# nanograv/PTMCMCSampler

Measured on AMD Instinct MI355X. Metric: MH updates/sec (whole node) + ESS/sec, 100-d Gaussian, 64 temps x 4096 walkers per GPU, higher is better.
Workload: dtype f64

## Files before the change

ptmcmcsampler_amd/csrc/ptmi_mh.inc.h:

```cpp
#pragma once
#include <stdlib.h>

#include "ptmi_common.h"

template <bool STR, int J>
__device__ __forceinline__ u64 grp_bcast(u64 v)
{
    if (STR) return (u64)__shfl((long long)v, (int)(threadIdx.x & 15) + 16 * J, 64);
    return quad_bcast<J>(v);
}
template <bool STR, int J>
__device__ __forceinline__ double grp_bcastf(double v)
{
    if (STR) return __shfl(v, (int)(threadIdx.x & 15) + 16 * J, 64);
    return quad_bcastf<J>(v);
}
template <int G, bool STR>
__device__ __forceinline__ double grp_sum(double p)
{
    if (STR) {
        p = p + __shfl_xor(p, 32, 64);
        p = p + __shfl_xor(p, 16, 64);
        return p;
    }
// ... 1092 lines not shown
    double cd_c = 0.0, cd_n = 0.0;

    constexpr bool PIPE = PAIRED && PERS != 0 && !FULL && !GRP && LOGL == PTMI_LOGL_ISO && PRI == PTMI_LOGP_FLAT;
    double x[EPL], dq[EPL], urow[PIPE ? EPL : 1];
#pragma unroll
    for (int e = 0; e < EPL; ++e) PTMI_ROW_LOAD(x[e], xrow, e);
    double lnL = a.lnL[ch], lp = a.lp[ch];
    u32 nacc = 0, jp[PTMI_J_FUSED] = {0, 0, 0}, ja[PTMI_J_FUSED] = {0, 0, 0};
    long long am_next = (FULL && a.am_base != nullptr) ? a.am_base[ch] : 0;
    const bool cold = live && tg == 0 && a.AM != nullptr;
    int am_row = a.am_row0;
    double box_margin = -1.0;
    double box_guard = 0.0;

    constexpr bool SQUAD = SCAMFAST && ScamBatch<STR, GW>::QUAD;
    constexpr bool PASSES = GW > 4 || SQUAD;
    constexpr int KPASS = GW > 4 ? GW / 2 : (SQUAD ? 4 : (1 << 30));
    constexpr int STM = (PERS || TLDS) ? 1 : (ULDS ? 2 : 0);
    auto scam_root_s = [&](int kk) {
        if (ULDS && !ulds_box) return smem[d * d + kk];
        return det_sqrt(S[kk]);
    };
    [[maybe_unused]] int koff = 0;
    [[maybe_unused]] auto row_request = [&](int off) __attribute__((always_inline)) {
        if constexpr (PIPE) {
            const double *row = smem + off;
            const ptmi_d2 *rp = reinterpret_cast<const ptmi_d2 *>(row) + gl;
#pragma unroll
            for (int e2 = 0; e2 < EPL / 2; ++e2) { const ptmi_d2 v = rp[4 * e2]; urow[2 * e2] = v.x; urow[2 * e2 + 1] = v.y; }
            if (EPL & 1) urow[EPL - 1] = row[8 * (EPL / 2) + gl];
        }
    };
    int kp = 0;
    if constexpr (PIPE) {
        for (; a.nsteps - kp >= 4; kp += 4) {
            sbatch.template refill<STM>(a, a.iter0 + kp, sid, gl, cc, d, [&](int kk) {
                const double rs = scam_root_s(kk);
                koff = kk * d;
                row_request((int)dpp32<0x00>((u32)koff));
                __builtin_amdgcn_sched_barrier(0);
                return rs;
            }, smem);
            {
                const int k = kp;
#define PTMI_STEP_S 0
#include "ptmi_mh_step.inc.h"
#undef PTMI_STEP_S
            }
            {
                const int k = kp + 1;
#define PTMI_STEP_S 1
#include "ptmi_mh_step.inc.h"
#undef PTMI_STEP_S
            }
            {
                const int k = kp + 2;
#define PTMI_STEP_S 2
#include "ptmi_mh_step.inc.h"
#undef PTMI_STEP_S
            }
            {
                const int k = kp + 3;
#define PTMI_STEP_S 3
#include "ptmi_mh_step.inc.h"
#undef PTMI_STEP_S
            }
        }
    }
    for (int k0 = PIPE ? kp : 0; k0 < a.nsteps; k0 += KPASS) {
    const int kend = (PASSES && a.nsteps - k0 > KPASS) ? k0 + KPASS : a.nsteps;
    if constexpr (GW > 4) {
        if constexpr (SCAMFAST) sbatch.template refill<0>(a, a.iter0 + k0, sid, gl, cc, d, [&](int kk) { return det_sqrt(S[kk]); }, nullptr);
        else batch.template refill<TM>(a, a.iter0 + k0, sid, gl, tsm);
    } else if constexpr (SQUAD) {
        sbatch.template refill<STM>(a, a.iter0 + k0, sid, gl, cc, d, scam_root_s, smem);
    }
    for (int k = k0; k < kend; ++k) {
#define PTMI_STEP_S (-1)
#include "ptmi_mh_step.inc.h"
#undef PTMI_STEP_S
    }
    }
    if (live) {
#pragma unroll
        for (int e = 0; e < EPL; ++e) {
            const int i = gl + G * e;
            if (e < safe_slots(G, EPL) || i < d) xrow[i] = x[e];
        }
        if (gl == 0) {
            a.lnL[ch] = lnL;
            a.lp[ch] = lp;
            const size_t r = (size_t)w * nt + t;
            a.nacc[r] += nacc;
            if (!FULL) { jp[PTMI_J_SCAM] = (u32)a.nsteps; ja[PTMI_J_SCAM] = nacc; }
#pragma unroll
            for (int j = 0; j < PTMI_J_FUSED; ++j) {
                a.jstat[(r * PTMI_J_NTYPES + j) * 2 + 0] += jp[j];
                a.jstat[(r * PTMI_J_NTYPES + j) * 2 + 1] += ja[j];
            }
        }
    }
    }
}

#ifndef PTMI_PC_PRIO
#define PTMI_PC_PRIO 0
#endif
#ifndef PTMI_PC_SPRIO
#define PTMI_PC_SPRIO 1
#endif
#ifndef PTMI_PC_ACCV
#define PTMI_PC_ACCV 1
// ... 738 lines not shown
```

ptmcmcsampler_amd/csrc/ptmi_mh_step.inc.h:

```cpp
#ifndef PTMI_STEP_S
#error "define PTMI_STEP_S (-1, or the step's index in a straight-line pass) before including ptmi_mh_step.inc.h"
#endif
        constexpr int SV = PTMI_STEP_S;
        const long long it = a.iter0 + k;
        if constexpr (AMQ) {
            if (amq_on) {
                const int s4 = k & 3, c16 = lane & 15;
                if (s4 == 0) {
                    auto look = [&](int kb, u64 &mask, int &rank, double &cdv, int base) {
                        bool ev = false;
                        cdv = 0.0;
                        if (kb + gl < a.nsteps) {
                            u64 p0, p1;
                            philox_words(a.seed, (u64)(a.iter0 + kb + gl), sid, 0u, p0, p1);
                            const int w_de = a.de_on ? a.w_de : 0;
                            const int ind = (int)h2index((u32)(p0 >> 32), (u32)(a.w_host + a.w_scam + a.w_am + w_de)) - a.w_host;
                            ev = live && ind >= a.w_scam && ind < a.w_scam + a.w_am;
                            constexpr u32 T97 = (u32)(0.97 * 4294967296.0), T90 = (u32)(0.9 * 4294967296.0);
                            const u32 plo = (u32)p0;
                            cdv = a.gcn[0] * cc.sc(plo > T97 ? 0 : (plo > T90 ? 1 : 2));
                        }
                        mask = __ballot(ev);
                        rank = base + (int)__popcll(mask & ((1ull << lane) - 1ull));
                        if (ev) PTMI_AMQ_IDX[rank & 127] = lane | (((kb >> 2) & 1) << 6);
                    };
                    if (k == 0) look(0, mask_n, rank_n, cd_n, 0);
                    mask_c = mask_n; rank_c = rank_n; cd_c = cd_n; base_c = base_n;
                    base_n = base_c + (int)__popcll(mask_c);
                    look(k + 4, mask_n, rank_n, cd_n, base_n);
                    asm volatile("" ::: "memory");
                }
                const int cons = base_c + (int)__popcll(mask_c & ((1ull << (16 * s4)) - 1ull));
                const int need = base_c + (int)__popcll(mask_c & (s4 == 3 ? ~0ull : ((1ull << (16 * s4 + 16)) - 1ull)));
                if (q_done < need) {
                    const int known = base_n + (int)__popcll(mask_n);
                    const int hi = known < cons + 16 ? known : cons + 16;
// ... 3 lines not shown
                    const int owner = entry & 63;
                    const bool of_cur = (entry >> 6) == ((k >> 2) & 1);
                    const u32 sid_ev = (u32)__shfl((int)sid, owner, 64);
                    const double cdc = __shfl(cd_c, owner, 64), cdn = __shfl(cd_n, owner, 64);
                    const double cd_ev = of_cur ? cdc : cdn;
                    const long long it_ev = a.iter0 + (k - s4) + (of_cur ? 0 : 4) + (owner >> 4);
                    MfmaAcc<EPL> acc;
                    if (UT_ALWAYS_LDS || a.lds_u) am_mfma_product<EPL>(a, valid, sid_ev, it_ev, cd_ev, d, PTMI_UL, true, mfma_ld(EPL), PTMI_SQ, true, acc, tsm);
                    else am_mfma_product<EPL>(a, valid, sid_ev, it_ev, cd_ev, d, UtBlock, false, d, PTMI_SQ, true, acc, tsm);
                    if (valid) {
#pragma unroll
                        for (int e = 0; e < EPL; ++e) PTMI_AMQ(r & 15)[gl * EPL + e] = acc.at(e);
                    }
                    q_done = hi;
                    asm volatile("" ::: "memory");
                }
            }
        }
        double log_u;
        int jt = PTMI_J_SCAM;
        double scam_amp = 0.0, box_reach = 0.0;
        if constexpr (SCAMFAST) {
            ScamDraw sd;
            if constexpr (SV >= 0) {
                constexpr int QP = (SV & 3) * 0x55;
                sd.log_u = dppf64<QP>(sbatch.lg);
                sd.amp = dppf64<QP>(sbatch.amp);
                sd.k = 0;
            } else {
                scam_draws_for_step<STR, STM, GW>(sbatch, sd, a, k, sid, gl, cc, d, scam_root_s, smem);
            }
            log_u = sd.log_u;
            if constexpr (SV >= 0) {
#pragma unroll
                for (int e = 0; e < EPL; ++e) dq[e] = sd.amp * urow[e];
                if constexpr (SV < 3) {
                    constexpr int QN = ((SV + 1) & 3) * 0x55;
                    __builtin_amdgcn_sched_barrier(0);
                    row_request((int)dpp32<QN>((u32)koff));
                    __builtin_amdgcn_sched_barrier(0);
                }
            } else if constexpr (PAIRED) {
                const double *row = smem + (size_t)sd.k * d;
                const ptmi_d2 *rp = reinterpret_cast<const ptmi_d2 *>(row) + gl;
#pragma unroll
                for (int e2 = 0; e2 < EPL / 2; ++e2) { const ptmi_d2 v = rp[4 * e2]; dq[2 * e2] = v.x; dq[2 * e2 + 1] = v.y; }
                if (EPL & 1) dq[EPL - 1] = row[8 * (EPL / 2) + gl];
            } else {
                if constexpr (ULDS) {
#pragma unroll
                    for (int e = 0; e < EPL; ++e) PTMI_ROW_LOAD(dq[e], smem + (size_t)sd.k * d, e);
                } else {
                    if constexpr (UPAD) {
                        const double *col = a.UtPad + (size_t)sd.k * (G * EPL) + gl;
                        constexpr int SPB = 512 / G;
#pragma unroll
                        for (int e = 0; e < EPL; ++e) {
                            const double *base = col + (e / SPB) * 512;
                            dq[e] = base[G * (e % SPB)];
                        }
                        __builtin_amdgcn_sched_barrier(0);
                    } else {
                        const double *col = UtBlock + (size_t)sd.k * d;
#pragma unroll
                        for (int e = 0; e < EPL; ++e) PTMI_ROW_LOAD(dq[e], col, e);
                    }
// ... 21 lines not shown
                for (int e = 0; e < EPL; ++e) dq[e] = PTMI_AMQ(rk & 15)[gl * EPL + e];
            }
        }
        if (FULL) {
#pragma unroll
            for (int j = 0; j < PTMI_J_FUSED; ++j) jp[j] += (jt == j);
        }
        double nlp, nlnL = 0.0, nlnprob;
        {
            double q[EPL];
#pragma unroll
            for (int e = 0; e < EPL; ++e) q[e] = x[e] + dq[e];
            if constexpr (PRI == PTMI_LOGP_FLAT) nlp = 0.0;
            else if constexpr (BOXFAST) {
                box_reach = __builtin_fabs(scam_amp) * box_umax;
                bool inside = box_reach < box_margin;
                if (!inside) {
                    bool in1;
                    double mg, bm;
                    box_test_and_margin<G, EPL>(smem, a.box_off, gl, x, dq, in1, mg, bm);
                    inside = grp_all<G, STR>(in1);
                    box_margin = grp_min<G, STR>(mg) * (1.0 - 0x1.0p-40);
                    box_guard = -grp_min<G, STR>(-bm) * 0x1.0p-52;
                }
                nlp = inside ? 0.0 : -__builtin_inf();
            }
            else if constexpr (PERS != 0 && PRI == PTMI_LOGP_BOX)
                nlp = grp_all<G, STR>(box_inside_lds<G, EPL>(smem, a.box_off, gl, [&](int e) { return q[e]; })) ? 0.0 : -__builtin_inf();
            else nlp = eval_logp<G, EPL, STR>(a, q, gl, smem);
            if (STAGE) nlnL = eval_logl<G, EPL, LOGL, STR>(a, q, gl, PTMI_PL);
            else nlnL = eval_logl<G, EPL, LOGL, STR>(a, q, gl, PtG);
            nlnprob = nlp == -__builtin_inf() ? -__builtin_inf() : beta * nlnL + nlp;
        }
        const double lnprob0 = beta * lnL + lp;
        const double diff = nlnprob - lnprob0 + 0.0;
        const bool accepted = diff > log_u;
        if (accepted) {
#pragma unroll
            for (int e = 0; e < EPL; ++e) {
                double inc = dq[e];
                asm volatile("" : "+v"(inc));
                x[e] = x[e] + inc;
            }
            lnL = nlnL;
            lp = nlp;
            nacc += 1;
            if (FULL) {
#pragma unroll
                for (int j = 0; j < PTMI_J_FUSED; ++j) ja[j] += (jt == j);
            }
            if constexpr (BOXFAST) box_margin = (box_margin - box_reach - box_guard) * (1.0 - 0x1.0p-40);
        }
        if (cold && !(a.swap_last && k == a.nsteps - 1)) {
            am_store_step<G, EPL>(a, w, am_row, k, x, gl, d, accepted);
            if (a.AMaux && gl == 0) {
                double *ax = a.AMaux + ((size_t)w * a.cov_update + (size_t)am_row) * 2;
                ax[0] = lnL;
                ax[1] = lp;
            }
        }
        am_row = am_row + 1 == a.cov_update ? 0 : am_row + 1;
```

ptmcmcsampler_amd/csrc/ptmi_abi.hip:

```cpp
#include <math.h>
#include <stdlib.h>

#include <new>
#include <vector>

#include <type_traits>

#include "ptmi_common.h"

static thread_local char g_err[512] = "";
int ptmi_fail(int code, const char *fmt, ...)
{
    va_list ap;
    va_start(ap, fmt);
    vsnprintf(g_err, sizeof(g_err), fmt, ap);
    va_end(ap);
    return code;
}

constexpr int WT = 7, WTILE = 16 * WT;
template <bool FUSED>
__global__ __launch_bounds__(256) void welford_kernel(const double *AM, double *mu, double *M2, double *cov, int d, int mem,
                                                     long long iter, int cov_stride_per_walker, int am_epl)
{
// ... 191 lines not shown
                if (u + 1 < RB) {
                    rd(u + 1, (u + 1) & 1);
                    __builtin_amdgcn_sched_barrier(0);
                }
                row(u & 1);
            }
        }
        __syncthreads();
    }
    if (!live) return;
    const double den = (double)(iter - 1);
    double *covw = cov ? cov + (size_t)w * cov_stride_per_walker : nullptr;
#pragma unroll
    for (int p = 0; p < PR; ++p)
#pragma unroll
        for (int r = 0; r < PC; ++r) {
            const int i = ty * PR + p, j = tx * PC + r;
            if (i < d && j < d) M2w[(size_t)i * d + j] = acc[p][r];
        }
    if (covw) {
#pragma unroll 1
        for (int e = 0; e < PR * PC; ++e) {
            const int i = ty * PR + e / PC, j = tx * PC + e % PC;
            if (i < d && j < d) covw[(size_t)i * d + j] = M2w[(size_t)i * d + j] / den;
        }
    }
}

constexpr int PS_W = 112;
constexpr int ps_rc(bool diag) { return diag ? 32 : 16; }
typedef double ps_d4 __attribute__((ext_vector_type(4)));
__host__ __device__ inline int pool_groups(int d) { return (d + 1 + PS_W - 1) / PS_W; }
static inline int pool_slab(int nwalkers, int d) { const int target = d + 1 <= PS_W ? 512 : 32; const int s = (nwalkers + target - 1) / target; return s < 1 ? 1 : s; }
struct PoolEnt { double wgt; int32_t src; int32_t pad; };
struct PoolRle { const PoolEnt *ent; const int32_t *cnt; };
typedef double ps_d2 __attribute__((ext_vector_type(2)));
constexpr int ps_nt(bool diag, int wv) { return diag ? 7 : (wv == 0 ? 13 : 12); }
__host__ __device__ constexpr int ps_t0(int wv) { return wv == 0 ? 0 : 1 + 12 * wv; }
constexpr int ps_ti(bool diag, int wv, int n) { return diag ? (n < 7 - wv ? wv : 7 - wv) : (ps_t0(wv) + n) / 7; }
constexpr int ps_tj(bool diag, int wv, int n) { return diag ? (n < 7 - wv ? wv + n : n) : (ps_t0(wv) + n) % 7; }
template <bool DIAG, int WV>
__device__ __forceinline__ void ps_mma(const double *Ab, const double *Bb, ps_d4 (&acc)[DIAG ? 7 : 13])
{
#pragma unroll
    for (int k0 = 0; k0 < ps_rc(DIAG); k0 += 4)
#pragma unroll
        for (int n = 0; n < ps_nt(DIAG, WV); ++n)
            acc[n] = __builtin_amdgcn_mfma_f64_16x16x4f64(Ab[k0 * PS_W + 16 * ps_ti(DIAG, WV, n)], Bb[k0 * PS_W + 16 * ps_tj(DIAG, WV, n)], acc[n], 0, 0, 0);
}
template <bool DIAG, int WV>
__device__ __forceinline__ void ps_store(const ps_d4 (&acc)[DIAG ? 7 : 13], double *out, int I, int J, int d, int am_epl, int g, int c)
{
#pragma unroll
    for (int n = 0; n < ps_nt(DIAG, WV); ++n) {
        const int ti = ps_ti(DIAG, WV, n), tj = ps_tj(DIAG, WV, n);
#pragma unroll
        for (int r = 0; r < 4; ++r) {
            const int pi = I * PS_W + 16 * ti + g + 4 * r, pj = J * PS_W + 16 * tj + c;
            if (pi < d && pj <= d && (!(DIAG && ti == tj) || pi <= pj)) {
                const int ci = am_inv(pi, am_epl), cj = pj < d ? am_inv(pj, am_epl) : d;
                const int lo = ci < cj ? ci : cj, hi = ci < cj ? cj : ci;
                out[(size_t)lo * (d + 1) + hi] = acc[n][r];
            }
        }
    }
}
template <bool DIAG, bool RLE, bool PAIR>
__global__ __launch_bounds__(256, 2) void pool_syrk_kernel(const double *rows, long long nrows, int d, const double *shift,
                                                                     long long rows_per_slab, double *part, int am_epl,
                                                                     int shift_epl ,
                                                                     PoolRle rl)
{
    constexpr int NTW = DIAG ? 7 : 13, NA = DIAG ? 1 : 2, PS_RC = ps_rc(DIAG), NU = PS_RC / 4;
    __shared__ double Dl[NA][2][PS_RC][PS_W];
    const int lane = (int)(threadIdx.x & 63), wave = __builtin_amdgcn_readfirstlane((int)(threadIdx.x >> 6));
    const int c = lane & 15, g = lane >> 4;
    const int ng = pool_groups(d);
    int I = (int)blockIdx.x, J = (int)blockIdx.x;
    if (!DIAG) {
        int p = (int)blockIdx.x;
        I = 0;
        while (p >= ng - 1 - I) { p -= ng - 1 - I; ++I; }
        J = I + 1 + p;
    }
    const long long beg = (long long)blockIdx.y * rows_per_slab;
    const int nlist = RLE ? rl.cnt[blockIdx.y] : (int)(beg + rows_per_slab < nrows ? rows_per_slab : nrows - beg);
    const char *slab = (const char *)(rows + beg * d);
    const PoolEnt *ent = RLE ? rl.ent + beg : nullptr;
    ps_d4 acc[NTW];
#pragma unroll
    for (int n = 0; n < NTW; ++n) acc[n] = ps_d4{0.0, 0.0, 0.0, 0.0};
    int offa[DIAG ? 1 : NTW], offb[DIAG ? 1 : NTW];
    if constexpr (!DIAG) {
#pragma unroll
        for (int n = 0; n < NTW; ++n) {
            const int t = ps_t0(wave) + n < 49 ? ps_t0(wave) + n : 48;
            offa[n] = __builtin_amdgcn_readfirstlane(16 * (t / 7));
            offb[n] = __builtin_amdgcn_readfirstlane(16 * (t % 7));
        }
    }
    const int q = 16 * wave + c, r4 = g;
    const bool stager = q < PS_W / 2;
    unsigned colb[NA][2];
    double sh[NA][2], one[NA][2];
    bool dat[NA][2];
    bool plain = true;
#pragma unroll
    for (int a2 = 0; a2 < NA; ++a2)
#pragma unroll
        for (int e = 0; e < 2; ++e) {
            const int p = (a2 == 0 ? I : J) * PS_W + 2 * q + e;
            dat[a2][e] = p < d;
            const int pc = PAIR ? (p - e < d ? p : d - 2 + e) : (p < d ? p : d - 1);
            colb[a2][e] = 8u * (unsigned)pc;
            sh[a2][e] = (stager && p < d) ? shift[am_pos(am_inv(p, am_epl), shift_epl)] : 0.0;
            one[a2][e] = p == d ? 1.0 : 0.0;
            plain = plain && (dat[a2][e] || !stager);
        }
    const bool wave_plain = __all(plain);
    const unsigned rstride = 8u * (unsigned)d;
    ps_d2 v[NA][NU];
    double wg[NU];
    int nsrc[RLE ? NU : 1];
    double nwg[RLE ? NU : 1];
    auto list = [&](int j0) {
        if constexpr (RLE) {
#pragma unroll
            for (int u = 0; u < NU; ++u) {
                const int j = j0 + 4 * u + r4, jc = j < nlist ? j : nlist - 1;
                const ps_d2 e2 = *(const ps_d2 *)(ent + jc);
                nwg[u] = e2.x;
                nsrc[u] = (int)(__double_as_longlong(e2.y) & 0xffffffffll);
            }
        }
    };
    auto fetch = [&](int j0) {
#pragma unroll
        for (int u = 0; u < NU; ++u) {
            const int j = j0 + 4 * u + r4, jc = j < nlist ? j : nlist - 1;
            const unsigned rb = (unsigned)(RLE ? nsrc[u] : jc) * rstride;
            wg[u] = j < nlist ? (RLE ? nwg[u] : 1.0) : 0.0;
#pragma unroll
            for (int a2 = 0; a2 < NA; ++a2) {
                if constexpr (PAIR) v[a2][u] = *(const ps_d2 *)(slab + (rb + colb[a2][0]));
                else {
                    v[a2][u].x = *(const double *)(slab + (rb + colb[a2][0]));
                    v[a2][u].y = *(const double *)(slab + (rb + colb[a2][1]));
                }
            }
        }
    };
    auto stage = [&](int buf) {
        if (!stager) return;
        if (wave_plain) {
#pragma unroll
            for (int a2 = 0; a2 < NA; ++a2)
#pragma unroll
                for (int u = 0; u < NU; ++u) {
                    ps_d2 x;
                    x.x = (v[a2][u].x - sh[a2][0]) * wg[u];
                    x.y = (v[a2][u].y - sh[a2][1]) * wg[u];
                    *(ps_d2 *)&Dl[a2][buf][4 * u + r4][2 * q] = x;
                }
        } else {
#pragma unroll
            for (int a2 = 0; a2 < NA; ++a2)
#pragma unroll
                for (int u = 0; u < NU; ++u) {
                    ps_d2 x;
                    x.x = (dat[a2][0] ? v[a2][u].x - sh[a2][0] : one[a2][0]) * wg[u];
                    x.y = (dat[a2][1] ? v[a2][u].y - sh[a2][1] : one[a2][1]) * wg[u];
                    *(ps_d2 *)&Dl[a2][buf][4 * u + r4][2 * q] = x;
                }
        }
    };
    if (nlist > 0) {
        list(0);
        fetch(0);
        list(PS_RC);
        stage(0);
    }
    __syncthreads();
    int buf = 0;
    for (int j0 = 0; j0 < nlist; j0 += PS_RC) {
        const bool more = j0 + PS_RC < nlist;
        if (more) {
            fetch(j0 + PS_RC);
            list(j0 + 2 * PS_RC);
        }
        const double *Ab = &Dl[0][buf][0][0] + g * PS_W + c, *Bb = &Dl[NA - 1][buf][0][0] + g * PS_W + c;
        if constexpr (DIAG) {
            switch (wave) {
            case 0: ps_mma<DIAG, 0>(Ab, Bb, acc); break;
            case 1: ps_mma<DIAG, 1>(Ab, Bb, acc); break;
            case 2: ps_mma<DIAG, 2>(Ab, Bb, acc); break;
            default: ps_mma<DIAG, 3>(Ab, Bb, acc); break;
            }
        } else {
#pragma unroll
            for (int k0 = 0; k0 < PS_RC; k0 += 4)
#pragma unroll
                for (int n = 0; n < NTW; ++n)
                    if (n < 12 || wave == 0) acc[n] = __builtin_amdgcn_mfma_f64_16x16x4f64(Ab[k0 * PS_W + offa[n]], Bb[k0 * PS_W + offb[n]], acc[n], 0, 0, 0);
        }
        if (more) stage(buf ^ 1);
        __syncthreads();
        buf ^= 1;
    }
    double *out = part + (size_t)blockIdx.y * d * (d + 1);
    if constexpr (DIAG) {
        switch (wave) {
        case 0: ps_store<DIAG, 0>(acc, out, I, J, d, am_epl, g, c); break;
        case 1: ps_store<DIAG, 1>(acc, out, I, J, d, am_epl, g, c); break;
        case 2: ps_store<DIAG, 2>(acc, out, I, J, d, am_epl, g, c); break;
        default: ps_store<DIAG, 3>(acc, out, I, J, d, am_epl, g, c); break;
        }
    } else {
#pragma unroll
        for (int n = 0; n < NTW; ++n) {
            if (!(n < 12 || wave == 0)) continue;
#pragma unroll
            for (int r = 0; r < 4; ++r) {
                const int pi = I * PS_W + offa[n] + g + 4 * r, pj = J * PS_W + offb[n] + c;
                if (pi < d && pj <= d) {
                    const int ci = am_inv(pi, am_epl), cj = pj < d ? am_inv(pj, am_epl) : d;
                    const int lo = ci < cj ? ci : cj, hi = ci < cj ? cj : ci;
                    out[(size_t)lo * (d + 1) + hi] = acc[n][r];
                }
            }
        }
    }
}

__global__ __launch_bounds__(256) void pool_rle_kernel(const AmFlag *flag, long long nrows, long long rows_per_slab, PoolEnt *ent, int32_t *cnt)
{
    constexpr int NG = 8;
    __shared__ int wsum[NG][4], base_s;
    const long long beg = (long long)blockIdx.x * rows_per_slab;
    const long long end = beg + rows_per_slab < nrows ? beg + rows_per_slab : nrows;
    const int lane = (int)(threadIdx.x & 63), wave = (int)(threadIdx.x >> 6);
    if (threadIdx.x == 0) base_s = 0;
    __syncthreads();
    for (long long r0 = beg; r0 < end; r0 += 256 * NG) {
        AmFlag f[NG];
#pragma unroll
        for (int u = 0; u < NG; ++u) { const long long r = r0 + 256 * u + threadIdx.x; f[u] = flag[r < end ? r : end - 1]; }
        unsigned long long m[NG];
#pragma unroll
        for (int u = 0; u < NG; ++u) {
            const long long r = r0 + 256 * u + threadIdx.x;
            m[u] = __ballot(r < end && (f[u] & (AMROW_NEW | AMROW_KEY)) != 0);
            if (lane == 0) wsum[u][wave] = (int)__popcll(m[u]);
        }
        __syncthreads();
        int off = base_s;
#pragma unroll
        for (int u = 0; u < NG; ++u) {
            const long long r = r0 + 256 * u + threadIdx.x;
            int mine = off + (int)__popcll(m[u] & ((1ull << lane) - 1ull));
            for (int k = 0; k < wave; ++k) mine += wsum[u][k];
            if ((m[u] >> lane) & 1ull) ent[beg + mine].src = (int32_t)(r - beg);
            off += wsum[u][0] + wsum[u][1] + wsum[u][2] + wsum[u][3];
        }
        __syncthreads();
        if (threadIdx.x == 0) base_s = off;
        __syncthreads();
    }
    const int n = base_s;
    if (threadIdx.x == 0) cnt[blockIdx.x] = n;
    for (int j0 = 0; j0 < n; j0 += 256 * NG) {
        int here[NG], next[NG];
#pragma unroll
        for (int u = 0; u < NG; ++u) {
            const int j = j0 + 256 * u + (int)threadIdx.x, jc = j < n ? j : n - 1;
            here[u] = ent[beg + jc].src;
            next[u] = jc + 1 < n ? ent[beg + jc + 1].src : (int)(end - beg);
        }
#pragma unroll
        for (int u = 0; u < NG; ++u) {
            const int j = j0 + 256 * u + (int)threadIdx.x;
            if (j < n) ent[beg + j].wgt = det_sqrt((double)((long long)next[u] - (long long)here[u]));
        }
    }
}

__global__ __launch_bounds__(128) void am_expand_kernel(double *AM, const AmFlag *flag, int d, int cu, int w0, long long it_lo, long long it_hi,
                                                        long long base)
{
    const int w = w0 + (int)blockIdx.x;
    const AmFlag *fw = flag + (size_t)w * cu;
    double *aw = AM + (size_t)w * cu * d;
    long long it0 = it_lo;
    while (it0 > base && !(fw[it0 % cu] & (AMROW_NEW | AMROW_KEY))) --it0;
    for (int i = (int)threadIdx.x; i < d; i += (int)blockDim.x) {
        double x = aw[(size_t)(it0 % cu) * d + i];
        for (long long it = it0 + 1; it <= it_hi; ++it) {
            const int ring = (int)(it % cu);
            if (fw[ring] & (AMROW_NEW | AMROW_KEY)) x = aw[(size_t)ring * d + i];
            else if (it >= it_lo) aw[(size_t)ring * d + i] = x;
        }
    }
}
__global__ void pool_reduce_kernel(const double *part, int nslab, int d, double *Tsum)
{
    const long long idx = (long long)blockIdx.x * blockDim.x + threadIdx.x;
    const int ld = d + 1;
    if (idx >= (long long)d * ld) return;
    const int i = (int)(idx / ld), j = (int)(idx % ld);
    if (j < i) return;
    const size_t st = (size_t)d * ld;
    double sum = 0.0;
    int s = 0;
    for (; s + 32 <= nslab; s += 32) {
        double v[32];
// ... 738 lines not shown
    } else if (gj) {
        const size_t nch = (size_t)c.nwalkers * c.ntemps, lanes = (size_t)s.G * s.EPL;
        const size_t nvec = (size_t)GJV_TOP + (size_t)GJL_VECS * (c.nuts_maxdepth + 1);
        hipError_t e3 = hipMalloc((void **)&h->d_gj_scr, sizeof(double) * nvec * lanes * nch);
        if (e3 == hipSuccess) e3 = hipMalloc((void **)&h->d_gj_scal, sizeof(double) * (size_t)GJS_SCALARS * (c.nuts_maxdepth + 1) * nch);
        const int cpw = 64 / s.G;
        long long solo = cpw > 1 ? (long long)ptmi_env("PTMI_GJ_SOLO", (double)(nch / 32 < 1024 ? nch / 32 : 1024)) : 0;
        if (solo > (long long)nch) solo = (long long)nch;
        if (solo < 0) solo = 0;
        h->gj_solo = (int)solo;
        if (e3 == hipSuccess) e3 = hipMalloc((void **)&h->d_gj_order, sizeof(int32_t) * (nch + (size_t)solo * cpw + cpw));
        if (e3 == hipSuccess) e3 = hipMalloc((void **)&h->d_gj_bucket, sizeof(int32_t) * 3 * GJ_BUCKETS);
        if (e3 != hipSuccess || (rc = upload(&h->d_gj_tab, c.gj_tab, 3LL * c.ndim * c.ndim))) {
            ptmi_destroy(h);
            return e3 != hipSuccess ? fail(PTMI_EHIP, "gradient-jump scratch: %s", hipGetErrorString(e3)) : rc;
        }
    }
    if (gj) {
        h->gj_diag = 1;
        for (long long i = 0; i < 3LL * c.ndim * c.ndim && h->gj_diag; ++i) {
            const long long r = (i / c.ndim) % c.ndim, col = i % c.ndim;
            if (r != col && c.gj_tab[i] != 0.0) h->gj_diag = 0;
        }
    }
    h->cfg.gj_tab = nullptr;
    h->cfg.ladder = h->cfg.temps_mh = h->cfg.logl_par = h->cfg.logp_par = h->cfg.group_mask = nullptr;
    h->cfg.group_size = nullptr;
    hipError_t e = hipMalloc((void **)&h->d_pre, PTMI_SWAP_PRE_BYTES * (size_t)c.nwalkers * c.ntemps_global);
    if (e == hipSuccess && !c.cov_per_walker && c.temp0 == 0) {
        const int SL = pool_slab(c.nwalkers, c.ndim), nslab = (c.nwalkers + SL - 1) / SL;
        e = hipMalloc((void **)&h->d_pool_part, sizeof(double) * (size_t)nslab * c.ndim * (c.ndim + 1));
        if (e == hipSuccess) e = hipMalloc((void **)&h->d_pool_T, sizeof(double) * (size_t)c.ndim * (c.ndim + 1));
        if (buf->AMflag) {
            const size_t nrows = (size_t)c.nwalkers * c.cov_update;
            if (e == hipSuccess) e = hipMalloc((void **)&h->d_rle_ent, sizeof(PoolEnt) * nrows);
            if (e == hipSuccess) e = hipMalloc((void **)&h->d_rle_cnt, sizeof(int32_t) * (size_t)nslab);
        }
    }
    const bool am_main = c.w_am > 0 && (c.ngroups > 1 || s.G > 4) && c.ndim <= 1024 && c.w_host == 0;
    const bool am_split = !am_main && buf->Q != nullptr && c.w_am > 0 && c.ndim <= 1024 && c.w_host == 0;
    if (e == hipSuccess && (am_main || am_split)) e = ptmi_am_scratch_alloc(h, am_main);
    if (e == hipSuccess) e = hipEventCreate(&h->ev0);
    if (e == hipSuccess) e = hipEventCreate(&h->ev1);
    if (e != hipSuccess) { ptmi_destroy(h); return fail(PTMI_EHIP, "create: %s", hipGetErrorString(e)); }
    *out = h;
    return PTMI_OK;
}

int ptmi_destroy(ptmi_handle h)
{
    if (!h) return PTMI_OK;
    (void)hipFree(h->d_ladder); (void)hipFree(h->d_temps); (void)hipFree(h->d_beta); (void)hipFree(h->d_loglpar); (void)hipFree(h->d_logppar);
    (void)hipFree(h->d_pre); (void)hipFree(h->d_xint); (void)hipFree(h->d_hop);
    if (h->h_hop) { (void)hipHostFree(h->h_hop); (void)hipEventDestroy(h->hop_ev); }
    (void)hipFree(h->d_gsize); (void)hipFree(h->d_gmask); (void)hipFree(h->d_gcn); (void)hipFree(h->d_gdiv); (void)hipFree(h->d_pool_part); (void)hipFree(h->d_pool_T);
    (void)hipFree(h->d_ql_scr); (void)hipFree(h->d_qlw_scr); (void)hipFree(h->d_qlg_scr); (void)hipFree(h->d_sy_scr); (void)hipFree(h->d_utpad);
    free(h->gsize_host);
    ptmi_dc_plan_free(h);
    if (h->h_sy_info) (void)hipHostFree(h->h_sy_info);
    (void)hipFree(h->d_rle_ent); (void)hipFree(h->d_rle_cnt);
    (void)hipFree(h->d_am_ev); (void)hipFree(h->d_am_count); (void)hipFree(h->d_am_base); (void)hipFree(h->d_am_inc);
    (void)hipFree(h->d_am_grp); (void)hipFree(h->d_am_perm); (void)hipFree(h->d_am_kbase); (void)hipFree(h->d_am_next); (void)hipFree(h->d_iter);
    if (h->h_gj_n) (void)hipHostFree(h->h_gj_n);
    (void)hipFree(h->d_cj_fun);
    if (h->h_cj_offs) (void)hipHostFree(h->h_cj_offs);
    if (h->h_sup_n) (void)hipHostFree(h->h_sup_n);
    (void)hipFree(h->d_gj_tab); (void)hipFree(h->d_gj_scr); (void)hipFree(h->d_gj_scal); (void)hipFree(h->d_gj_order); (void)hipFree(h->d_gj_bucket);
    if (h->side) { (void)hipStreamDestroy(h->side); (void)hipEventDestroy(h->side_go); (void)hipEventDestroy(h->side_done); }
// ... 404 lines not shown
{
    if (!hh) return fail(PTMI_EINVAL, "NULL handle");
    ptmi_engine view = *hh;
    if (stream) view.stream = (hipStream_t)stream;
    if (AM_in) { view.buf.AM = const_cast<double *>(AM_in); view.buf.AMflag = const_cast<uint64_t *>(AMflag_in); }
    ptmi_engine *h = &view;
    struct Back { ptmi_engine *to, *from; ~Back() { to->side = from->side; to->side_go = from->side_go; to->side_done = from->side_done; } } back{hh, h};
    const ptmi_config &c = h->cfg;
    if (c.temp0 != 0) return PTMI_OK;
    if (!h->buf.AM || !h->buf.mu || !h->buf.M2 || !h->buf.cov) return fail(PTMI_EINVAL, "AM/mu/M2/cov buffers missing");
    if (iter < c.cov_update || iter % c.cov_update) return fail(PTMI_EINVAL, "iter must be a positive multiple of cov_update");
    const int d = c.ndim, nt = (d + WTILE - 1) / WTILE;
    if (c.cov_per_walker) {
        if (d <= 100)
            hipLaunchKernelGGL((welford_rows_kernel<25, 10, 4, 10>), dim3((c.nwalkers + 1) / 2), dim3(768), 0, h->stream, (const double *)h->buf.AM,
                               h->buf.mu, h->buf.M2, h->buf.cov, d, c.cov_update, (long long)iter, d * d, am_row_epl(h->G, h->EPL), c.nwalkers);
        else
        hipLaunchKernelGGL(welford_kernel<false>, dim3(nt, nt, c.nwalkers), dim3(256), 0, h->stream, (const double *)h->buf.AM,
                           h->buf.mu, h->buf.M2, h->buf.cov, d, c.cov_update, (long long)iter, d * d, am_row_epl(h->G, h->EPL));
        if (nt > 1)
            hipLaunchKernelGGL(welford_mean_kernel, dim3((d + 63) / 64, c.nwalkers), dim3(64), 0, h->stream, (const double *)h->buf.AM,
                               h->buf.mu, d, c.cov_update, (long long)iter, 0, am_row_epl(h->G, h->EPL));
    } else {
        const int W = c.nwalkers, SL = pool_slab(W, d), nslab = (W + SL - 1) / SL, ng = pool_groups(d);
        const long long nrows = (long long)W * c.cov_update;
        const bool first = iter == c.cov_update;
        const double *shift = first ? (const double *)h->buf.AM : (const double *)h->buf.mu;
        hipStream_t diag_stream = h->stream;
        const bool rle = h->buf.AMflag != nullptr, pair = d % 2 == 0;
        const PoolRle pr = {(const PoolEnt *)h->d_rle_ent, h->d_rle_cnt};
        const long long rps = (long long)SL * c.cov_update;
        if (rps * d * 8 >= (1ll << 32)) return fail(PTMI_EUNSUPPORTED, "pooled statistics: a slab of %d walkers x %d rows x %d parameters exceeds 4 GB", SL, c.cov_update, d);
        const int aepl = am_row_epl(h->G, h->EPL), sepl = first ? am_row_epl(h->G, h->EPL) : 0;
        if (rle) hipLaunchKernelGGL(pool_rle_kernel, dim3(nslab), dim3(256), 0, h->stream, (const AmFlag *)h->buf.AMflag, nrows, rps, (PoolEnt *)h->d_rle_ent,
                                    h->d_rle_cnt);
        auto syrk = [&](auto diag, dim3 grid, hipStream_t st) {
            constexpr bool DG = decltype(diag)::value;
            const void *fn = rle ? (pair ? (const void *)pool_syrk_kernel<DG, true, true> : (const void *)pool_syrk_kernel<DG, true, false>)
                                 : (pair ? (const void *)pool_syrk_kernel<DG, false, true> : (const void *)pool_syrk_kernel<DG, false, false>);
            const double *rows = (const double *)h->buf.AM;
            long long nr = nrows, rp = rps;
            int dd = d, ae = aepl, se = sepl;
            double *part = h->d_pool_part;
            PoolRle prl = pr;
            void *args[] = {&rows, &nr, &dd, (void *)&shift, &rp, &part, &ae, &se, &prl};
            return hipLaunchKernel(fn, grid, dim3(256), args, 0, st);
        };
        if (ng > 1) {
            if (!h->side) {
                HIPCHK(hipStreamCreateWithFlags(&h->side, hipStreamNonBlocking));
                HIPCHK(hipEventCreateWithFlags(&h->side_go, hipEventDisableTiming));
                HIPCHK(hipEventCreateWithFlags(&h->side_done, hipEventDisableTiming));
            }
            HIPCHK(hipEventRecord(h->side_go, h->stream));
            HIPCHK(hipStreamWaitEvent(h->side, h->side_go, 0));
            HIPCHK(syrk(std::false_type{}, dim3(ng * (ng - 1) / 2, nslab), h->stream));
            diag_stream = h->side;
        }
        HIPCHK(syrk(std::true_type{}, dim3(ng, nslab), diag_stream));
        if (ng > 1) {
            HIPCHK(hipEventRecord(h->side_done, h->side));
            HIPCHK(hipStreamWaitEvent(h->stream, h->side_done, 0));
        }
        const long long nel = (long long)d * (d + 1);
        hipLaunchKernelGGL(pool_reduce_kernel, dim3((unsigned)((nel + 63) / 64)), dim3(64), 0, h->stream, (const double *)h->d_pool_part, nslab, d,
                           h->d_pool_T);
        const double nb = (double)W * (double)c.cov_update, nprev = (double)W * (double)(iter - c.cov_update);
        hipLaunchKernelGGL(pool_finish_kernel, dim3((unsigned)(((long long)d * d + 255) / 256)), dim3(256), 0, h->stream, (const double *)h->d_pool_T,
// ... 123 lines not shown
```

Baseline: 35.50 billion.

## Specialize pipelined MH passes on wave-uniform cold flag and cache current log-probability

Wraps the 4-step pipelined SCAM loop in a lambda instantiated twice. The choice is made by a wave-wide ballot of `cold`, so hot-only waves compile out the adaptive-Metropolis row store and the am_row bookkeeping. The current beta*lnL+lp is carried in `lnprob_cur` and updated only on acceptance, instead of being recomputed every step. An explicit s_waitcnt is added before consuming the prefetched row. x is copied into a local array through asm moves to steer register allocation. Risks: am_row no longer advances in non-cold waves during these passes, the extra waitcnt may serialize loads, and the doubled code size adds instruction-cache pressure.

```diff
diff --git a/ptmcmcsampler_amd/csrc/ptmi_mh.inc.h b/ptmcmcsampler_amd/csrc/ptmi_mh.inc.h
--- a/ptmcmcsampler_amd/csrc/ptmi_mh.inc.h
+++ b/ptmcmcsampler_amd/csrc/ptmi_mh.inc.h
@@ -1148,40 +1148,62 @@
         }
     };
     int kp = 0;
+    [[maybe_unused]] double lnprob_cur = 0.0;
     if constexpr (PIPE) {
-        for (; a.nsteps - kp >= 4; kp += 4) {
-            sbatch.template refill<STM>(a, a.iter0 + kp, sid, gl, cc, d, [&](int kk) {
-                const double rs = scam_root_s(kk);
-                koff = kk * d;
-                row_request((int)dpp32<0x00>((u32)koff));
-                __builtin_amdgcn_sched_barrier(0);
-                return rs;
-            }, smem);
-            {
-                const int k = kp;
+        lnprob_cur = beta * lnL + lp;
+#define PTMI_STEP_AMROW COLDU
+        auto full_passes = [&](auto unit_has_cold) __attribute__((always_inline)) {
+            constexpr bool COLDU = decltype(unit_has_cold)::value;
+            double (&xu)[EPL] = x;
+            double x[EPL];
+#pragma unroll
+            for (int e = 0; e < EPL; ++e) {
+                if constexpr (COLDU) x[e] = xu[e];
+                else asm volatile("v_mov_b64 %0, %1" : "=v"(x[e]) : "v"(xu[e]));
+            }
+            for (; a.nsteps - kp >= 4; kp += 4) {
+                sbatch.template refill<STM>(a, a.iter0 + kp, sid, gl, cc, d, [&](int kk) {
+                    const double rs = scam_root_s(kk);
+                    koff = kk * d;
+                    row_request((int)dpp32<0x00>((u32)koff));
+                    __builtin_amdgcn_sched_barrier(0);
+                    return rs;
+                }, smem);
+                {
+                    const int k = kp;
 #define PTMI_STEP_S 0
 #include "ptmi_mh_step.inc.h"
 #undef PTMI_STEP_S
-            }
-            {
-                const int k = kp + 1;
+                }
+                {
+                    const int k = kp + 1;
 #define PTMI_STEP_S 1
 #include "ptmi_mh_step.inc.h"
 #undef PTMI_STEP_S
-            }
-            {
-                const int k = kp + 2;
+                }
+                {
+                    const int k = kp + 2;
 #define PTMI_STEP_S 2
 #include "ptmi_mh_step.inc.h"
 #undef PTMI_STEP_S
-            }
-            {
-                const int k = kp + 3;
+                }
+                {
+                    const int k = kp + 3;
 #define PTMI_STEP_S 3
 #include "ptmi_mh_step.inc.h"
 #undef PTMI_STEP_S
-            }
-        }
+                }
+            }
+#pragma unroll
+            for (int e = 0; e < EPL; ++e) {
+                if constexpr (COLDU) xu[e] = x[e];
+                else asm volatile("v_mov_b64 %0, %1" : "=v"(xu[e]) : "v"(x[e]));
+            }
+        };
+#undef PTMI_STEP_AMROW
+        const bool unit_cold = __ballot(cold) != 0ull;
+        if (unit_cold) full_passes(std::true_type{});
+        else full_passes(std::false_type{});
     }
     for (int k0 = PIPE ? kp : 0; k0 < a.nsteps; k0 += KPASS) {
     const int kend = (PASSES && a.nsteps - k0 > KPASS) ? k0 + KPASS : a.nsteps;
@@ -1193,7 +1215,9 @@
     }
     for (int k = k0; k < kend; ++k) {
 #define PTMI_STEP_S (-1)
+#define PTMI_STEP_AMROW true
 #include "ptmi_mh_step.inc.h"
+#undef PTMI_STEP_AMROW
 #undef PTMI_STEP_S
     }
     }
diff --git a/ptmcmcsampler_amd/csrc/ptmi_mh_step.inc.h b/ptmcmcsampler_amd/csrc/ptmi_mh_step.inc.h
--- a/ptmcmcsampler_amd/csrc/ptmi_mh_step.inc.h
+++ b/ptmcmcsampler_amd/csrc/ptmi_mh_step.inc.h
@@ -1,7 +1,11 @@
 #ifndef PTMI_STEP_S
 #error "define PTMI_STEP_S (-1, or the step's index in a straight-line pass) before including ptmi_mh_step.inc.h"
 #endif
+#ifndef PTMI_STEP_AMROW
+#error "define PTMI_STEP_AMROW (true, or a compile-time bool of the pass loop) before including ptmi_mh_step.inc.h"
+#endif
         constexpr int SV = PTMI_STEP_S;
+        constexpr bool AMROW = PTMI_STEP_AMROW;
         const long long it = a.iter0 + k;
         if constexpr (AMQ) {
             if (amq_on) {
@@ -71,6 +75,9 @@
             }
             log_u = sd.log_u;
             if constexpr (SV >= 0) {
+                __builtin_amdgcn_sched_barrier(0);
+                __builtin_amdgcn_s_waitcnt(0xc07f);
+                __builtin_amdgcn_sched_barrier(0);
 #pragma unroll
                 for (int e = 0; e < EPL; ++e) dq[e] = sd.amp * urow[e];
                 if constexpr (SV < 3) {
@@ -158,8 +165,14 @@
             else nlnL = eval_logl<G, EPL, LOGL, STR>(a, q, gl, PtG);
             nlnprob = nlp == -__builtin_inf() ? -__builtin_inf() : beta * nlnL + nlp;
         }
-        const double lnprob0 = beta * lnL + lp;
-        const double diff = nlnprob - lnprob0 + 0.0;
+        double lnprob0, diff;
+        if constexpr (SV >= 0) {
+            lnprob0 = lnprob_cur;
+            diff = nlnprob - lnprob0;
+        } else {
+            lnprob0 = beta * lnL + lp;
+            diff = nlnprob - lnprob0 + 0.0;
+        }
         const bool accepted = diff > log_u;
         if (accepted) {
 #pragma unroll
@@ -170,6 +183,7 @@
             }
             lnL = nlnL;
             lp = nlp;
+            if constexpr (SV >= 0) lnprob_cur = nlnprob;
             nacc += 1;
             if (FULL) {
 #pragma unroll
@@ -177,12 +191,14 @@
             }
             if constexpr (BOXFAST) box_margin = (box_margin - box_reach - box_guard) * (1.0 - 0x1.0p-40);
         }
-        if (cold && !(a.swap_last && k == a.nsteps - 1)) {
-            am_store_step<G, EPL>(a, w, am_row, k, x, gl, d, accepted);
-            if (a.AMaux && gl == 0) {
-                double *ax = a.AMaux + ((size_t)w * a.cov_update + (size_t)am_row) * 2;
-                ax[0] = lnL;
-                ax[1] = lp;
-            }
-        }
-        am_row = am_row + 1 == a.cov_update ? 0 : am_row + 1;
+        if constexpr (AMROW) {
+            if (cold && !(a.swap_last && k == a.nsteps - 1)) {
+                am_store_step<G, EPL>(a, w, am_row, k, x, gl, d, accepted);
+                if (a.AMaux && gl == 0) {
+                    double *ax = a.AMaux + ((size_t)w * a.cov_update + (size_t)am_row) * 2;
+                    ax[0] = lnL;
+                    ax[1] = lp;
+                }
+            }
+            am_row = am_row + 1 == a.cov_update ? 0 : am_row + 1;
+        }
```

New measurement: 35.81 billion, median of 6. Within noise of the previous version (+0.9%).

## Precompute RLE byte offsets, specialize syrk kernel per wave, parallelize RLE build per walker

Applied to the files above, without the earlier changes.

The pooled-covariance syrk kernel is split into a per-wave templated body, so tile indices become compile-time constants and the runtime offset arrays and switch statements go away. RLE entries now carry a precomputed byte offset and are padded per slab with zero-weight tail entries, which lets the fetch skip index clamping. A non-RLE fast path loads full chunks without bounds checks. The RLE build kernel is rewritten to work per walker with wave-level ballots and a reverse scan, computing weights in one pass instead of a second sweep. Costs are more template instantiations, higher register pressure risk, and a 32-bit offset limit.

```diff
diff --git a/ptmcmcsampler_amd/csrc/ptmi_abi.hip b/ptmcmcsampler_amd/csrc/ptmi_abi.hip
--- a/ptmcmcsampler_amd/csrc/ptmi_abi.hip
+++ b/ptmcmcsampler_amd/csrc/ptmi_abi.hip
@@ -247,7 +247,7 @@
 typedef double ps_d4 __attribute__((ext_vector_type(4)));
 __host__ __device__ inline int pool_groups(int d) { return (d + 1 + PS_W - 1) / PS_W; }
 static inline int pool_slab(int nwalkers, int d) { const int target = d + 1 <= PS_W ? 512 : 32; const int s = (nwalkers + target - 1) / target; return s < 1 ? 1 : s; }
-struct PoolEnt { double wgt; int32_t src; int32_t pad; };
+struct alignas(16) PoolEnt { double wgt; int32_t src; uint32_t off; };
 struct PoolRle { const PoolEnt *ent; const int32_t *cnt; };
 typedef double ps_d2 __attribute__((ext_vector_type(2)));
 constexpr int ps_nt(bool diag, int wv) { return diag ? 7 : (wv == 0 ? 13 : 12); }
@@ -280,15 +280,14 @@
         }
     }
 }
-template <bool DIAG, bool RLE, bool PAIR>
-__global__ __launch_bounds__(256, 2) void pool_syrk_kernel(const double *rows, long long nrows, int d, const double *shift,
-                                                                     long long rows_per_slab, double *part, int am_epl,
-                                                                     int shift_epl ,
-                                                                     PoolRle rl)
+__host__ __device__ inline int pool_ent_padded(int n) { return ((n + 31) / 32 + 1) * 32; }
+__host__ __device__ inline long long pool_ent_stride(long long rows_per_slab) { return ((rows_per_slab + 31) / 32 + 1) * 32; }
+template <bool DIAG, bool RLE, bool PAIR, int WV>
+__device__ __forceinline__ void ps_wave(double (&Dl)[DIAG ? 1 : 2][2][ps_rc(DIAG)][PS_W], const double *rows, long long nrows, int d,
+                                        const double *shift, long long rows_per_slab, double *part, int am_epl, int shift_epl, PoolRle rl)
 {
     constexpr int NTW = DIAG ? 7 : 13, NA = DIAG ? 1 : 2, PS_RC = ps_rc(DIAG), NU = PS_RC / 4;
-    __shared__ double Dl[NA][2][PS_RC][PS_W];
-    const int lane = (int)(threadIdx.x & 63), wave = __builtin_amdgcn_readfirstlane((int)(threadIdx.x >> 6));
+    const int lane = (int)(threadIdx.x & 63), wave = WV;
     const int c = lane & 15, g = lane >> 4;
     const int ng = pool_groups(d);
     int I = (int)blockIdx.x, J = (int)blockIdx.x;
@@ -301,19 +300,9 @@
     const long long beg = (long long)blockIdx.y * rows_per_slab;
     const int nlist = RLE ? rl.cnt[blockIdx.y] : (int)(beg + rows_per_slab < nrows ? rows_per_slab : nrows - beg);
     const char *slab = (const char *)(rows + beg * d);
-    const PoolEnt *ent = RLE ? rl.ent + beg : nullptr;
     ps_d4 acc[NTW];
 #pragma unroll
     for (int n = 0; n < NTW; ++n) acc[n] = ps_d4{0.0, 0.0, 0.0, 0.0};
-    int offa[DIAG ? 1 : NTW], offb[DIAG ? 1 : NTW];
-    if constexpr (!DIAG) {
-#pragma unroll
-        for (int n = 0; n < NTW; ++n) {
-            const int t = ps_t0(wave) + n < 49 ? ps_t0(wave) + n : 48;
-            offa[n] = __builtin_amdgcn_readfirstlane(16 * (t / 7));
-            offb[n] = __builtin_amdgcn_readfirstlane(16 * (t % 7));
-        }
-    }
     const int q = 16 * wave + c, r4 = g;
     const bool stager = q < PS_W / 2;
     unsigned colb[NA][2];
@@ -336,32 +325,52 @@
     const unsigned rstride = 8u * (unsigned)d;
     ps_d2 v[NA][NU];
     double wg[NU];
-    int nsrc[RLE ? NU : 1];
-    double nwg[RLE ? NU : 1];
+    unsigned noff[RLE ? NU : 1];
+    const PoolEnt *ent = RLE ? rl.ent + (long long)blockIdx.y * pool_ent_stride(rows_per_slab) : nullptr;
+    const size_t eoff = sizeof(PoolEnt) * (size_t)r4;
     auto list = [&](int j0) {
         if constexpr (RLE) {
+            const char *ec = (const char *)(ent + j0) + eoff;
+#pragma unroll
+            for (int u = 0; u < NU; ++u) noff[u] = ((const PoolEnt *)(ec + 4 * sizeof(PoolEnt) * u))->off;
+        }
+    };
+    unsigned rowb[NA][2];
+#pragma unroll
+    for (int a2 = 0; a2 < NA; ++a2)
+#pragma unroll
+        for (int e = 0; e < 2; ++e) rowb[a2][e] = (unsigned)r4 * rstride + colb[a2][e];
+    auto load = [&](int a2, int u, const char *base, unsigned rb, const unsigned (&cb)[NA][2]) {
+        if constexpr (PAIR) v[a2][u] = *(const ps_d2 *)(base + (rb + cb[a2][0]));
+        else {
+            v[a2][u].x = *(const double *)(base + (rb + cb[a2][0]));
+            v[a2][u].y = *(const double *)(base + (rb + cb[a2][1]));
+        }
+    };
+    auto fetch = [&](int j0) {
+        if constexpr (RLE) {
+            const char *ec = (const char *)(ent + j0) + eoff;
+#pragma unroll
+            for (int u = 0; u < NU; ++u) {
+                wg[u] = ((const PoolEnt *)(ec + 4 * sizeof(PoolEnt) * u))->wgt;
+#pragma unroll
+                for (int a2 = 0; a2 < NA; ++a2) load(a2, u, slab, noff[u], colb);
+            }
+        } else if (j0 + PS_RC <= nlist) {
+#pragma unroll
+            for (int u = 0; u < NU; ++u) {
+                const char *base = slab + (size_t)(j0 + 4 * u) * rstride;
+                wg[u] = 1.0;
+#pragma unroll
+                for (int a2 = 0; a2 < NA; ++a2) load(a2, u, base, 0u, rowb);
+            }
+        } else {
 #pragma unroll
             for (int u = 0; u < NU; ++u) {
                 const int j = j0 + 4 * u + r4, jc = j < nlist ? j : nlist - 1;
-                const ps_d2 e2 = *(const ps_d2 *)(ent + jc);
-                nwg[u] = e2.x;
-                nsrc[u] = (int)(__double_as_longlong(e2.y) & 0xffffffffll);
-            }
-        }
-    };
-    auto fetch = [&](int j0) {
-#pragma unroll
-        for (int u = 0; u < NU; ++u) {
-            const int j = j0 + 4 * u + r4, jc = j < nlist ? j : nlist - 1;
-            const unsigned rb = (unsigned)(RLE ? nsrc[u] : jc) * rstride;
-            wg[u] = j < nlist ? (RLE ? nwg[u] : 1.0) : 0.0;
-#pragma unroll
-            for (int a2 = 0; a2 < NA; ++a2) {
-                if constexpr (PAIR) v[a2][u] = *(const ps_d2 *)(slab + (rb + colb[a2][0]));
-                else {
-                    v[a2][u].x = *(const double *)(slab + (rb + colb[a2][0]));
-                    v[a2][u].y = *(const double *)(slab + (rb + colb[a2][1]));
-                }
+                wg[u] = j < nlist ? 1.0 : 0.0;
+#pragma unroll
+                for (int a2 = 0; a2 < NA; ++a2) load(a2, u, slab, (unsigned)jc * rstride, colb);
             }
         }
     };
@@ -404,97 +413,114 @@
             list(j0 + 2 * PS_RC);
         }
         const double *Ab = &Dl[0][buf][0][0] + g * PS_W + c, *Bb = &Dl[NA - 1][buf][0][0] + g * PS_W + c;
-        if constexpr (DIAG) {
-            switch (wave) {
-            case 0: ps_mma<DIAG, 0>(Ab, Bb, acc); break;
-            case 1: ps_mma<DIAG, 1>(Ab, Bb, acc); break;
-            case 2: ps_mma<DIAG, 2>(Ab, Bb, acc); break;
-            default: ps_mma<DIAG, 3>(Ab, Bb, acc); break;
-            }
-        } else {
-#pragma unroll
-            for (int k0 = 0; k0 < PS_RC; k0 += 4)
-#pragma unroll
-                for (int n = 0; n < NTW; ++n)
-                    if (n < 12 || wave == 0) acc[n] = __builtin_amdgcn_mfma_f64_16x16x4f64(Ab[k0 * PS_W + offa[n]], Bb[k0 * PS_W + offb[n]], acc[n], 0, 0, 0);
-        }
+        ps_mma<DIAG, WV>(Ab, Bb, acc);
         if (more) stage(buf ^ 1);
         __syncthreads();
         buf ^= 1;
     }
     double *out = part + (size_t)blockIdx.y * d * (d + 1);
-    if constexpr (DIAG) {
-        switch (wave) {
-        case 0: ps_store<DIAG, 0>(acc, out, I, J, d, am_epl, g, c); break;
-        case 1: ps_store<DIAG, 1>(acc, out, I, J, d, am_epl, g, c); break;
-        case 2: ps_store<DIAG, 2>(acc, out, I, J, d, am_epl, g, c); break;
-        default: ps_store<DIAG, 3>(acc, out, I, J, d, am_epl, g, c); break;
-        }
-    } else {
-#pragma unroll
-        for (int n = 0; n < NTW; ++n) {
-            if (!(n < 12 || wave == 0)) continue;
-#pragma unroll
-            for (int r = 0; r < 4; ++r) {
-                const int pi = I * PS_W + offa[n] + g + 4 * r, pj = J * PS_W + offb[n] + c;
-                if (pi < d && pj <= d) {
-                    const int ci = am_inv(pi, am_epl), cj = pj < d ? am_inv(pj, am_epl) : d;
-                    const int lo = ci < cj ? ci : cj, hi = ci < cj ? cj : ci;
-                    out[(size_t)lo * (d + 1) + hi] = acc[n][r];
+    ps_store<DIAG, WV>(acc, out, I, J, d, am_epl, g, c);
+}
+template <bool DIAG, bool RLE, bool PAIR>
+__global__ __launch_bounds__(256, 2) void pool_syrk_kernel(const double *rows, long long nrows, int d, const double *shift,
+                                                                     long long rows_per_slab, double *part, int am_epl,
+                                                                     int shift_epl ,
+                                                                     PoolRle rl)
+{
+    __shared__ double Dl[DIAG ? 1 : 2][2][ps_rc(DIAG)][PS_W];
+    switch (__builtin_amdgcn_readfirstlane((int)(threadIdx.x >> 6))) {
+    case 0: ps_wave<DIAG, RLE, PAIR, 0>(Dl, rows, nrows, d, shift, rows_per_slab, part, am_epl, shift_epl, rl); break;
+    case 1: ps_wave<DIAG, RLE, PAIR, 1>(Dl, rows, nrows, d, shift, rows_per_slab, part, am_epl, shift_epl, rl); break;
+    case 2: ps_wave<DIAG, RLE, PAIR, 2>(Dl, rows, nrows, d, shift, rows_per_slab, part, am_epl, shift_epl, rl); break;
+    default: ps_wave<DIAG, RLE, PAIR, 3>(Dl, rows, nrows, d, shift, rows_per_slab, part, am_epl, shift_epl, rl); break;
+    }
+}
+
+constexpr int PR_WAVES = 8;
+__global__ __launch_bounds__(64 * PR_WAVES) void pool_rle_kernel(const AmFlag *flag, int nwalkers, int cu, int walkers_per_slab, int d, PoolEnt *ent,
+                                                                 int32_t *cnt)
+{
+    constexpr int NB = 16;
+    constexpr int NR = 256;
+    __shared__ int wcnt[NR];
+    const int lane = (int)(threadIdx.x & 63), wave = __builtin_amdgcn_readfirstlane((int)(threadIdx.x >> 6));
+    const int w_beg = (int)blockIdx.x * walkers_per_slab;
+    const int nw = walkers_per_slab < nwalkers - w_beg ? walkers_per_slab : nwalkers - w_beg;
+    PoolEnt *se = ent + (long long)blockIdx.x * pool_ent_stride((long long)walkers_per_slab * cu);
+    const int ngr = (cu + 63) / 64;
+    const unsigned rstride = 8u * (unsigned)d;
+    auto total = [&](int n) {
+        int s = 0;
+        for (int t = lane; t < n; t += 64) s += wcnt[t];
+#pragma unroll
+        for (int m = 32; m >= 1; m >>= 1) s += __shfl_xor(s, m, 64);
+        return __builtin_amdgcn_readfirstlane(s);
+    };
+    int base = 0;
+    for (int i0 = 0; i0 < nw; i0 += NR) {
+        const int nr = nw - i0 < NR ? nw - i0 : NR;
+        for (int i = wave; i < nr; i += PR_WAVES) {
+            const AmFlag *fw = flag + (size_t)(w_beg + i0 + i) * cu;
+            int n = 0;
+            for (int k0 = 0; k0 < ngr; k0 += NB) {
+                AmFlag f[NB];
+#pragma unroll
+                for (int u = 0; u < NB; ++u) { const int r = 64 * (k0 + u) + lane; f[u] = fw[r < cu ? r : cu - 1]; }
+#pragma unroll
+                for (int u = 0; u < NB; ++u) {
+                    const int r = 64 * (k0 + u) + lane;
+                    n += (int)__popcll(__ballot(r < cu && (f[u] & (AMROW_NEW | AMROW_KEY)) != 0));
                 }
             }
-        }
-    }
-}
-
-__global__ __launch_bounds__(256) void pool_rle_kernel(const AmFlag *flag, long long nrows, long long rows_per_slab, PoolEnt *ent, int32_t *cnt)
-{
-    constexpr int NG = 8;
-    __shared__ int wsum[NG][4], base_s;
-    const long long beg = (long long)blockIdx.x * rows_per_slab;
-    const long long end = beg + rows_per_slab < nrows ? beg + rows_per_slab : nrows;
-    const int lane = (int)(threadIdx.x & 63), wave = (int)(threadIdx.x >> 6);
-    if (threadIdx.x == 0) base_s = 0;
-    __syncthreads();
-    for (long long r0 = beg; r0 < end; r0 += 256 * NG) {
-        AmFlag f[NG];
-#pragma unroll
-        for (int u = 0; u < NG; ++u) { const long long r = r0 + 256 * u + threadIdx.x; f[u] = flag[r < end ? r : end - 1]; }
-        unsigned long long m[NG];
-#pragma unroll
-        for (int u = 0; u < NG; ++u) {
-            const long long r = r0 + 256 * u + threadIdx.x;
-            m[u] = __ballot(r < end && (f[u] & (AMROW_NEW | AMROW_KEY)) != 0);
-            if (lane == 0) wsum[u][wave] = (int)__popcll(m[u]);
+            if (lane == 0) wcnt[i] = n;
         }
         __syncthreads();
-        int off = base_s;
-#pragma unroll
-        for (int u = 0; u < NG; ++u) {
-            const long long r = r0 + 256 * u + threadIdx.x;
-            int mine = off + (int)__popcll(m[u] & ((1ull << lane) - 1ull));
-            for (int k = 0; k < wave; ++k) mine += wsum[u][k];
-            if ((m[u] >> lane) & 1ull) ent[beg + mine].src = (int32_t)(r - beg);
-            off += wsum[u][0] + wsum[u][1] + wsum[u][2] + wsum[u][3];
-        }
-        __syncthreads();
-        if (threadIdx.x == 0) base_s = off;
-        __syncthreads();
-    }
-    const int n = base_s;
-    if (threadIdx.x == 0) cnt[blockIdx.x] = n;
-    for (int j0 = 0; j0 < n; j0 += 256 * NG) {
-        int here[NG], next[NG];
-#pragma unroll
-        for (int u = 0; u < NG; ++u) {
-            const int j = j0 + 256 * u + (int)threadIdx.x, jc = j < n ? j : n - 1;
-            here[u] = ent[beg + jc].src;
-            next[u] = jc + 1 < n ? ent[beg + jc + 1].src : (int)(end - beg);
-        }
-#pragma unroll
-        for (int u = 0; u < NG; ++u) {
-            const int j = j0 + 256 * u + (int)threadIdx.x;
-            if (j < n) ent[beg + j].wgt = det_sqrt((double)((long long)next[u] - (long long)here[u]));
+        for (int i = wave; i < nr; i += PR_WAVES) {
+            const AmFlag *fw = flag + (size_t)(w_beg + i0 + i) * cu;
+            const int first = base + total(i), mine = wcnt[i];
+            const int row0 = (i0 + i) * cu;
+            int above = 0, nxt = cu, last = 0;
+            for (int k0 = (ngr - 1) / NB * NB; k0 >= 0; k0 -= NB) {
+                AmFlag f[NB];
+#pragma unroll
+                for (int u = 0; u < NB; ++u) { const int r = 64 * (k0 + u) + lane; f[u] = fw[r < cu ? r : cu - 1]; }
+#pragma unroll
+                for (int u = NB - 1; u >= 0; --u) {
+                    const int r = 64 * (k0 + u) + lane;
+                    const unsigned long long m = __ballot(r < cu && (f[u] & (AMROW_NEW | AMROW_KEY)) != 0);
+                    const int nm = (int)__popcll(m);
+                    if ((m >> lane) & 1ull) {
+                        const unsigned long long higher = (m >> lane) >> 1;
+                        const int next = higher ? r + 1 + (int)__builtin_ctzll(higher) : nxt;
+                        const int j = first + mine - above - nm + (int)__popcll(m & ((1ull << lane) - 1ull));
+                        PoolEnt e;
+                        e.wgt = det_sqrt((double)(next - r));
+                        e.src = row0 + r;
+                        e.off = (uint32_t)(row0 + r) * rstride;
+                        se[j] = e;
+                    }
+                    if (m) {
+                        if (above == 0) last = 64 * (k0 + u) + 63 - (int)__builtin_clzll(m);
+                        nxt = 64 * (k0 + u) + (int)__builtin_ctzll(m);
+                        above += nm;
+                    }
+                }
+            }
+            if (i0 + i == nw - 1) {
+                const int n = first + mine;
+                if (lane == 0) cnt[blockIdx.x] = n;
+                if (lane < pool_ent_padded(n) - n) {
+                    PoolEnt e;
+                    e.wgt = 0.0;
+                    e.src = row0 + last;
+                    e.off = (uint32_t)(row0 + last) * rstride;
+                    se[n + lane] = e;
+                }
+            }
+        }
+        if (i0 + NR < nw) {
+            base += total(nr);
+            __syncthreads();
         }
     }
 }
@@ -1299,8 +1325,7 @@
         e = hipMalloc((void **)&h->d_pool_part, sizeof(double) * (size_t)nslab * c.ndim * (c.ndim + 1));
         if (e == hipSuccess) e = hipMalloc((void **)&h->d_pool_T, sizeof(double) * (size_t)c.ndim * (c.ndim + 1));
         if (buf->AMflag) {
-            const size_t nrows = (size_t)c.nwalkers * c.cov_update;
-            if (e == hipSuccess) e = hipMalloc((void **)&h->d_rle_ent, sizeof(PoolEnt) * nrows);
+            if (e == hipSuccess) e = hipMalloc((void **)&h->d_rle_ent, sizeof(PoolEnt) * (size_t)nslab * (size_t)pool_ent_stride((long long)SL * c.cov_update));
             if (e == hipSuccess) e = hipMalloc((void **)&h->d_rle_cnt, sizeof(int32_t) * (size_t)nslab);
         }
     }
@@ -1771,8 +1796,8 @@
         const long long rps = (long long)SL * c.cov_update;
         if (rps * d * 8 >= (1ll << 32)) return fail(PTMI_EUNSUPPORTED, "pooled statistics: a slab of %d walkers x %d rows x %d parameters exceeds 4 GB", SL, c.cov_update, d);
         const int aepl = am_row_epl(h->G, h->EPL), sepl = first ? am_row_epl(h->G, h->EPL) : 0;
-        if (rle) hipLaunchKernelGGL(pool_rle_kernel, dim3(nslab), dim3(256), 0, h->stream, (const AmFlag *)h->buf.AMflag, nrows, rps, (PoolEnt *)h->d_rle_ent,
-                                    h->d_rle_cnt);
+        if (rle) hipLaunchKernelGGL(pool_rle_kernel, dim3(nslab), dim3(64 * PR_WAVES), 0, h->stream, (const AmFlag *)h->buf.AMflag, W, c.cov_update, SL, d,
+                                    (PoolEnt *)h->d_rle_ent, h->d_rle_cnt);
         auto syrk = [&](auto diag, dim3 grid, hipStream_t st) {
             constexpr bool DG = decltype(diag)::value;
             const void *fn = rle ? (pair ? (const void *)pool_syrk_kernel<DG, true, true> : (const void *)pool_syrk_kernel<DG, true, false>)
```

Measured after the change: 35.62 billion before, 35.81 billion after, median of 6. Within noise of the previous version (+0.5%).
